# Jarvis73/PEMP

Measured on AMD Instinct MI355X. Metric: episodes/sec (PEMP stage-1 eval step, PASCAL-5i-shaped 1-shot, ResNet-50), higher is better.
Workload: dtype f32

## Files before the change

### pemp_amd/csrc/conv_common.h

```cpp
#pragma once
#include "common.h"

namespace pemp {

typedef __attribute__((ext_vector_type(16))) float f32x16;
typedef __attribute__((ext_vector_type(4))) float v4f;
typedef __attribute__((ext_vector_type(8))) __bf16 bf16x8;
typedef __attribute__((ext_vector_type(2))) unsigned int u32x2;

#define PEMP_CONV_BF16_IO 0x100u

__device__ __forceinline__ v4f load_quad(const float* base, size_t off, unsigned bf16) {
    if (!bf16) return *(const v4f*)(base + off);
    const u32x2 r = *(const u32x2*)((const unsigned short*)base + off);
    return v4f{__builtin_bit_cast(float, r.x << 16), __builtin_bit_cast(float, r.x & 0xFFFF0000u),
               __builtin_bit_cast(float, r.y << 16), __builtin_bit_cast(float, r.y & 0xFFFF0000u)};
}

__device__ __forceinline__ unsigned int bf16_bits(float f) {
    const unsigned int u = __builtin_bit_cast(unsigned int, f);
    if ((u & 0x7FFFFFFFu) > 0x7F800000u) return (u >> 16) | 0x40u;
    return (u + 0x7FFFu + ((u >> 16) & 1u)) >> 16;
}

// ... 224 lines not shown
                o.y = fmaxf(o.y, 0.f);
                o.z = fmaxf(o.z, 0.f);
                o.w = fmaxf(o.w, 0.f);
            }
            store_quad(a.y, (size_t)m * a.ldy + n, o, a.flags & PEMP_CONV_BF16_IO);
        }
    }
}

int launch_conv_dma(int tile, const ConvArgs& a, hipStream_t st);
bool conv_dma2_supported(const ConvArgs& a);
int launch_conv_dma2(int tile, const ConvArgs& a, hipStream_t st);
int launch_conv_dma2_group(int tile, ConvGroupArgs& g, hipStream_t st);
int launch_conv_dma2_hybrid(const ConvArgs& a, hipStream_t st);
int conv_dma2_hybrid_rows(int M, int Cout);
int launch_conv_dma2_bf16(int tile, const ConvArgs& a, hipStream_t st);
int launch_conv_dma2_db(int tile, ConvArgs a, void* ws, size_t ws_bytes, bool split, hipStream_t st);
int conv_dma2_tile_rows(int tile);
struct SplitKPlan { int full, split, pieces; size_t ws_bytes; };
SplitKPlan conv_dma2_splitk_plan(int tile, const ConvArgs& a);
int launch_conv_dma2_splitk(int tile, ConvArgs a, void* ws, size_t ws_bytes, hipStream_t st);
int launch_conv_dma2_split3(int tile, ConvArgs a, void* ws, size_t ws_bytes, bool split, hipStream_t st);
int launch_conv_dma2_group_split3(int tile, ConvGroupArgs& g, hipStream_t st);
int pack_split3(const float* w, void* out, int cout, int kpad, hipStream_t st);

}
```

### pemp_amd/csrc/conv_dma2.hip

```cpp
#include "conv_common.h"

#ifndef PEMP_SK_ACQUIRE
#define PEMP_SK_ACQUIRE 1
#endif

namespace pemp {

typedef __attribute__((address_space(3))) void* lptr_t;

template <int BM, int BN, int WGM, int NW, bool PADV, int EPI = 0, bool SK = false, bool BF16 = false, bool DB = false, bool R16 = false,
          bool S3 = false>
__device__ __forceinline__ void conv_dma2_body(const ConvArgs& a, const int bid, const int nblk) {
#if defined(__HIP_DEVICE_COMPILE__)
    constexpr int WGN = NW / WGM;
    constexpr int RPI = NW * 8;
    constexpr int WM = BM / WGM, WN = BN / WGN;
    static_assert(!R16 || (WM == 16 && WN % 16 == 0 && EPI == 0 && !SK && !BF16 && !DB), "R16: 16-row wave tiles, plain epilogue only");
    static_assert(!S3 || (EPI == 0 && !BF16 && !DB && !R16), "S3: plain epilogue, fp32 operands");
    constexpr int TM = R16 ? 1 : WM / 32, TN = R16 ? WN / 16 : WN / 32;
    constexpr int BQ = S3 ? 12 : 8;
    static_assert(!S3 || (BN * BQ) % (NW * 64) == 0, "S3: whole B DMA rounds");
    constexpr int AL = BM / RPI, BL = S3 ? BN * BQ / (NW * 64) : BN / RPI;
    constexpr int NMF = S3 ? 6 * TM * TN : R16 ? 2 * TN : TM * TN * (BF16 ? 1 : 4), NDS = S3 ? 2 * TM + 3 * TN : R16 ? 1 + TN : TM + TN,
                  NDMA = AL + BL;
// ... 211 lines not shown
                acc[mi][ni] = __builtin_amdgcn_mfma_f32_32x32x16_bf16(am_[mi], bm_, acc[mi][ni], 0, 0, 0);        \
                acc[mi][ni] = __builtin_amdgcn_mfma_f32_32x32x16_bf16(am_[mi], bh_, acc[mi][ni], 0, 0, 0);        \
                acc[mi][ni] = __builtin_amdgcn_mfma_f32_32x32x16_bf16(ah_[mi], bm_, acc[mi][ni], 0, 0, 0);        \
                acc[mi][ni] = __builtin_amdgcn_mfma_f32_32x32x16_bf16(ah_[mi], bh_, acc[mi][ni], 0, 0, 0);        \
            }                                                                                                     \
        } else if constexpr (R16) {        \
            _Pragma("unroll") for (int h_ = 0; h_ < 2; ++h_) _Pragma("unroll") for (int ni = 0; ni < TN; ++ni)    \
                acc16[ni] = __builtin_amdgcn_mfma_f32_16x16x4f32(a16[src_][h_], b16[src_][ni][h_], acc16[ni], 0, 0, 0); \
        } else                                                                                                    \
        _Pragma("unroll") for (int mi = 0; mi < TM; ++mi) _Pragma("unroll") for (int ni = 0; ni < TN; ++ni) {     \
            const v4f av = af[src_][mi], bv = bf[src_][ni];                                                       \
            if constexpr (BF16) {                                                                                 \
                acc[mi][ni] = __builtin_amdgcn_mfma_f32_32x32x16_bf16(__builtin_bit_cast(bf16x8, av),              \
                                                                      __builtin_bit_cast(bf16x8, bv), acc[mi][ni], 0, 0, 0); \
                continue;                                                                                         \
            }                                                                                                     \
            acc[mi][ni] = __builtin_amdgcn_mfma_f32_32x32x2f32(av.x, bv.x, acc[mi][ni], 0, 0, 0);                 \
            acc[mi][ni] = __builtin_amdgcn_mfma_f32_32x32x2f32(av.y, bv.y, acc[mi][ni], 0, 0, 0);                 \
            acc[mi][ni] = __builtin_amdgcn_mfma_f32_32x32x2f32(av.z, bv.z, acc[mi][ni], 0, 0, 0);                 \
            acc[mi][ni] = __builtin_amdgcn_mfma_f32_32x32x2f32(av.w, bv.w, acc[mi][ni], 0, 0, 0);                 \
        }                                                                                                         \
    } while (0)

#define PEMP_STEP(buf_, DMA_, NEXT_)                                                                              \
    do {                                                                                                          \
        PEMP_READ(1, buf_, 1);                                                                                    \
        __builtin_amdgcn_sched_barrier(0);                                                                        \
        PEMP_MMA(0);                                                                                              \
        __builtin_amdgcn_sched_barrier(0);                                                                        \
        if constexpr (!S3) {                                         \
            PEMP_READ(0, buf_, 2);                                                                                \
            __builtin_amdgcn_sched_barrier(0);                                                                    \
            PEMP_MMA(1);                                                                                          \
            __builtin_amdgcn_sched_barrier(0);                                                                    \
            PEMP_READ(1, buf_, 3);                                                                                \
            __builtin_amdgcn_sched_barrier(0);                                                                    \
            PEMP_MMA(0);                                                                                          \
            __builtin_amdgcn_sched_barrier(0);                                                                    \
        }                                                                                                         \
          \
        __builtin_amdgcn_s_waitcnt(0x0070);           \
        asm volatile("s_waitcnt vmcnt(0)" ::: "memory");       \
        __builtin_amdgcn_s_barrier();    \
        __builtin_amdgcn_sched_barrier(0);                                                                        \
        if (NEXT_) PEMP_READ(0, (buf_) ^ 1, 0);                                                                   \
        if (DMA_) {                                                                                               \
            PEMP_ADVANCE2();                                                                                      \
            PEMP_DMA2(buf_);                                                                                      \
        }                                                                                                         \
        PEMP_MMA(1);                          \
        if (DMA_) {                         \
            _Pragma("unroll") for (int k_ = 0; k_ < NMF; ++k_) {                                                  \
                __builtin_amdgcn_sched_group_barrier(0x008, 1, 0);                                                \
                _Pragma("unroll") for (int q_ = 0; q_ < PER; ++q_) {                                              \
                    const int it_ = k_ * PER + q_;                                                                \
                    if (it_ < NDS) __builtin_amdgcn_sched_group_barrier(0x100, 1, 0);                             \
                    else if (it_ < NDS + NDMA) __builtin_amdgcn_sched_group_barrier(0x020, 1, 0);                 \
                }                                                                                                 \
            }                                                                                                     \
        }                                                                                                         \
        __builtin_amdgcn_sched_barrier(0);                                                                        \
    } while (0)

    int kt = 0;
    PEMP_READ(0, 0, 0);
    for (; kt + 2 < nkl; ++kt) {
        const int buf = kt & 1;
        PEMP_STEP(buf, true, true);
    }
    if (kt + 1 < nkl) {
// ... 3 lines not shown
    }
    constexpr bool PRE = !R16 && TM * TN <= 2;
    v4f rpre[PRE ? TM * TN * 4 : 1];
#pragma unroll
    for (int i = 0; i < (PRE ? TM * TN * 4 : 1); ++i) rpre[i] = v4f{0.f, 0.f, 0.f, 0.f};
    if constexpr (PRE) {
        if (a.res) {
            const int rr_ = lane >> 3, c4_ = (lane & 7) * 4;
#pragma unroll
            for (int mi = 0; mi < TM; ++mi)
#pragma unroll
                for (int ni = 0; ni < TN; ++ni)
#pragma unroll
                    for (int i = 0; i < 4; ++i) {
                        const int m = m0 + wm0 + mi * 32 + rr_ + 8 * i, n = n0 + wn0 + ni * 32 + c4_;
                        rpre[(mi * TN + ni) * 4 + i] = m < a.M ? load_quad(a.res, (size_t)m * a.ldr + n, a.flags & PEMP_CONV_BF16_IO) : v4f{0.f, 0.f, 0.f, 0.f};
                    }
        }
    }
    {
        const int buf = kt & 1;
        PEMP_STEP(buf, false, false);
    }
#undef PEMP_STEP
#undef PEMP_DMA2
#undef PEMP_ADVANCE2
#undef PEMP_READ
#undef PEMP_MMA

    if constexpr (SK) {
        if (sk_r >= 0) {
            v4f* part = (v4f*)a.sk_ws + ((size_t)(sk_r * a.sk_S + piece) * NW + wave) * (TM * TN * 4 * 64) + lane;
#pragma unroll
            for (int mi = 0; mi < TM; ++mi)
#pragma unroll
                for (int ni = 0; ni < TN; ++ni)
#pragma unroll
                    for (int q = 0; q < 4; ++q) {
                        const v4f v = {acc[mi][ni][4 * q], acc[mi][ni][4 * q + 1], acc[mi][ni][4 * q + 2], acc[mi][ni][4 * q + 3]};
                        asm volatile("global_store_dwordx4 %0, %1, off sc0 sc1" ::"v"(part + ((mi * TN + ni) * 4 + q) * 64), "v"(v) : "memory");
                    }
            asm volatile("s_waitcnt vmcnt(0)" ::: "memory");
            __syncthreads();
            int* flag = (int*)smem;
            if (tid == 0) {
                const int v = __hip_atomic_fetch_add(a.sk_cnt + sk_r, 1, __ATOMIC_RELAXED, __HIP_MEMORY_SCOPE_AGENT);
#if PEMP_SK_ACQUIRE
                if (v == a.sk_S - 1) {
                    __builtin_amdgcn_fence(__ATOMIC_ACQUIRE, "agent");
                    asm volatile("s_waitcnt vmcnt(0)" ::: "memory");
                }
// ... 60 lines not shown

    float* Rall = (float*)smem + NW * 1024;
    static_assert(EPI == 0 || NW * 1024 + NW * TN * 512 <= 64 * (BM + BN), "LDS: statistics area");
    static_assert(NW * 1024 <= 64 * (BM + BN), "LDS: one 4 KB transpose patch per wave");
    if constexpr (R16) conv_epilogue_r16<TN>(a, acc16, (float*)smem + wave * 1024, m0 + wm0, n0 + wn0, lane);
    else if constexpr (PRE) conv_epilogue_lds_pre<TM, TN, TM * TN * 4, EPI, DB>(a, acc, (float*)smem + wave * 1024, m0 + wm0, n0 + wn0, lane, rpre, Rall + wave * TN * 512);
    else if constexpr (EPI != 0) {
        const v4f none[1] = {{0.f, 0.f, 0.f, 0.f}};
        conv_epilogue_lds_pre<TM, TN, 1, EPI>(a, acc, (float*)smem + wave * 1024, m0 + wm0, n0 + wn0, lane, none, Rall + wave * TN * 512);
    } else conv_epilogue_lds<TM, TN, DB>(a, acc, (float*)smem + wave * 1024, m0 + wm0, n0 + wn0, lane);
    if constexpr (EPI != 0) {
        __syncthreads();
        conv_stats_store<BN, WGM, NW, TN>(a, Rall, bm, n0, tid);
    }
#endif
}

template <int BM, int BN, int WGM, int NW, bool PADV, int EPI = 0, bool SK = false, bool BF16 = false, bool DB = false, bool R16 = false,
          bool S3 = false>
__global__ __launch_bounds__(NW * 64) void conv_dma2_kernel(ConvArgs a) {
    conv_dma2_body<BM, BN, WGM, NW, PADV, EPI, SK, BF16, DB, R16, S3>(a, blockIdx.x, gridDim.x);
}

template <int BM, int BN, int WGM, int NW, bool PADV, bool R16 = false, bool S3 = false>
__global__ __launch_bounds__(NW * 64) void conv_dma2_group_kernel(ConvGroupArgs g) {
    int which = 0;
#pragma unroll
    for (int i = 1; i < CONV_GROUP_MAX; ++i) which += (i < g.n && (int)blockIdx.x >= g.first[i]) ? 1 : 0;
    const int bid = (int)blockIdx.x - g.first[which];
    if (bid >= g.nblk[which]) return;
    conv_dma2_body<BM, BN, WGM, NW, PADV, 0, false, false, false, R16, S3>(g.a[which], bid, g.nblk[which]);
}

template <int BM, int BN, int WGM, int NW, bool R16 = false, bool S3 = false>
static int launch_dma2_group(ConvGroupArgs& g, bool padv, hipStream_t st) {
    const size_t lds = (size_t)2 * (8 * BM + (S3 ? 12 : 8) * BN) * sizeof(v4f);
    auto kern = padv ? conv_dma2_group_kernel<BM, BN, WGM, NW, true, R16, S3> : conv_dma2_group_kernel<BM, BN, WGM, NW, false, R16, S3>;
    if (lds > 64 * 1024) {
        hipError_t e = hipFuncSetAttribute((const void*)kern, hipFuncAttributeMaxDynamicSharedMemorySize, (int)lds);
        if (e != hipSuccess) {
            set_error("hipFuncSetAttribute(lds=%zu): %s", lds, hipGetErrorString(e));
            return (int)e;
        }
    }
    int grid = 0;
    for (int i = 0; i < g.n; ++i) {
        g.first[i] = grid;
        g.nblk[i] = cdiv(g.a[i].M, BM) * (g.a[i].Cout / BN);
        grid += (g.nblk[i] + 7) & ~7;
    }
    g.first[g.n] = grid;
    hipLaunchKernelGGL(kern, dim3(grid), dim3(NW * 64), lds, st, g);
    return launch_status("conv_dma2/group");
}

static int g_simds_of[64] = {0};

template <bool PADV>
__global__ __launch_bounds__(256) void conv_dma2_hybrid_kernel(ConvGroupArgs g) {
    const int bid = (int)blockIdx.x;
    if (bid < g.first[1]) {
        if (bid < g.nblk[0]) conv_dma2_body<64, 64, 2, 4, PADV, 0, false, false, false, false>(g.a[0], bid, g.nblk[0]);
    } else {
        conv_dma2_body<32, 64, 2, 4, PADV, 0, false, false, false, true>(g.a[1], bid - g.first[1], g.nblk[1]);
    }
}

int conv_dma2_hybrid_rows(int M, int Cout) {
    int dev = 0;
    if (hipGetDevice(&dev) != hipSuccess || dev < 0 || dev >= 64) dev = 63;
    if (!g_simds_of[dev]) {
        int cus = 0;
        if (dev == 63 || hipDeviceGetAttribute(&cus, hipDeviceAttributeMultiprocessorCount, dev) != hipSuccess || cus <= 0) cus = 256;
        g_simds_of[dev] = 4 * cus;
    }
    const int g_simds = g_simds_of[dev];
    if (M <= 0 || Cout < 64 || Cout % 64) return 0;
    const int per32 = Cout / 32;
    const int rounds = (int)(((long long)M / 32 * per32) / g_simds);
    if (rounds < 1 || rounds > 8) return 0;
    const int rows_a = ((long long)rounds * g_simds / per32) * 32 / 64 * 64;
    const int rest = M - rows_a;
    if (rows_a <= 0 || rest <= 0 || (long long)cdiv(rest, 16) * per32 > g_simds) return 0;
    return rows_a;
}

int launch_conv_dma2_hybrid(const ConvArgs& a, hipStream_t st) {
    if (a.stats || (a.flags & PEMP_CONV_BF16_IO)) return -2;
    const int rows_a = conv_dma2_hybrid_rows(a.M, a.Cout);
    if (!rows_a) return -2;
    const int rest = a.M - rows_a;
    ConvGroupArgs g;
    g.n = 2;
    g.a[0] = a;
    g.a[0].M = rows_a;
    g.a[1] = a;
    g.a[1].bm_first = rows_a / 32;
    for (int i = 2; i < CONV_GROUP_MAX; ++i) g.a[i] = a;
    g.nblk[0] = (rows_a / 64) * (a.Cout / 64);
// ... 206 lines not shown
    if (tile < 1 || tile > 6 || tile == 5 || a.stats || a.rowmask || (a.flags & PEMP_CONV_BF16_IO)) {
        set_error("conv split3: tile %d / epilogue outside the family", tile);
        return -1;
    }
    int bm, bn;
    tile_shape(tile, bm, bn);
    if (split) {
        const SplitKPlan p = conv_dma2_splitk_plan(tile, a);
        if (p.pieces >= 2) {
            if (!ws || ws_bytes < p.ws_bytes || ((uintptr_t)ws & 15)) {
                set_error("conv split-K: workspace of %zu bytes needed (16-byte aligned), got %zu", p.ws_bytes, ws_bytes);
                return -1;
            }
            a.sk_cnt = (int*)ws;
            a.sk_ws = (float*)((char*)ws + 1024);
            a.sk_full = p.full;
            a.sk_S = p.pieces;
            return launch_s3_tile<true>(tile, a, p.full + p.split * p.pieces, st);
        }
    }
    return launch_s3_tile<false>(tile, a, cdiv(a.M, bm) * (a.Cout / bn), st);
}

int launch_conv_dma2_group_split3(int tile, ConvGroupArgs& g, hipStream_t st) {
    if (tile == 5) {
        set_error("conv split3: no 128 x 64 8-wave form");
        return -1;
    }
    const bool padv = g.a[0].padv != nullptr;
    if (tile == 6) return launch_dma2_group<256, 128, 8, 8, false, true>(g, padv, st);
    if (tile == 4) return launch_dma2_group<128, 128, 4, 8, false, true>(g, padv, st);
    if (tile == 1) return launch_dma2_group<128, 128, 4, 4, false, true>(g, padv, st);
    if (tile == 2) return launch_dma2_group<128, 64, 4, 4, false, true>(g, padv, st);
    return launch_dma2_group<64, 64, 2, 4, false, true>(g, padv, st);
}

__global__ __launch_bounds__(256) void pack_split3_kernel(const float* __restrict__ w, unsigned short* __restrict__ out, long long n8) {
    const long long i = (long long)blockIdx.x * 256 + threadIdx.x;
    if (i >= n8) return;
    const v4f x0 = *(const v4f*)(w + i * 8), x1 = *(const v4f*)(w + i * 8 + 4);
    bf16x8 h, m, l;
    split3_bf16(x0, x1, h, m, l);
    const long long step = i >> 2;
    unsigned short* o = out + step * 96 + (i & 3) * 8;
    *(bf16x8*)o = h;
    *(bf16x8*)(o + 32) = m;
// ... 49 lines not shown
```

### pemp_amd/csrc/conv_igemm.hip

```cpp
#include "conv_common.h"

namespace pemp {


template <int BM, int BN, int WGM, bool STEM>
__global__ __launch_bounds__(256) void conv_igemm_kernel(ConvArgs a) {
    constexpr int WGN = 4 / WGM;
    constexpr int WM = BM / WGM, WN = BN / WGN;
    constexpr int TM = WM / 32, TN = WN / 32;
    constexpr int AL = BM / 32, BL = BN / 32;
    static_assert(TM >= 1 && TN >= 1, "wave tile");

    extern __shared__ __attribute__((aligned(16))) v4f smem[];
    v4f* As = smem;
    v4f* Bs = smem + 2 * 8 * BM;

    const int tid = threadIdx.x;
    const int lane = tid & 63;
    const int wave = tid >> 6;
    const int wm0 = (wave / WGN) * WM;
    const int wn0 = (wave % WGN) * WN;
    const int lr = lane & 31, lh = lane >> 5;

    const int ntn = a.Cout / BN;
// ... 258 lines not shown
    a.dil = d->dil; a.ldr = d->ldr; a.Kpad = d->Kpad; a.flags = d->flags;
    a.HoWo = d->Ho * d->Wo;
    a.M = d->N * a.HoWo;
    a.ntaps = ntaps;
    a.cin_steps = stem ? 1 : d->Cin / 32;
    a.nk = d->Kpad / 32;
    if (residual) PEMP_REQUIRE(d->ldr >= d->Cout && d->ldr % 4 == 0 && ((uintptr_t)residual & 15) == 0, "conv2d: ldr must be >= Cout and x4, residual 16-byte aligned");
    a.sk_ws = nullptr; a.sk_cnt = nullptr; a.sk_full = 0; a.sk_S = 1;
    a.bm_first = 0;
    return 0;
}

static int conv2d_impl(const pemp_conv_desc* d, const float* x, const float* w, float* y, const float* scale, const float* shift,
                       const float* residual, const float* pad_value, void* ws, size_t ws_bytes, void* stream) {
    ConvArgs a;
    const int rc = conv_fill(d, x, w, y, scale, shift, residual, pad_value, a);
    if (rc) return rc;
    const bool stem = d->flags & PEMP_CONV_STEM4;
    int tile = d->tile;
    if (tile == 0) {
        tile = 3;
    }
    hipStream_t st = (hipStream_t)stream;
    if ((tile >= 41 && tile <= 46) || (tile >= 51 && tile <= 56)) {
        PEMP_REQUIRE(tile != 53, "conv2d: no split-K variant of the 64 x 64 tile");
        PEMP_REQUIRE(tile != 45 && tile != 55, "conv2d: no split3 form of the 128 x 64 8-wave tile");
        PEMP_REQUIRE(!stem && conv_dma2_supported(a) && (long long)a.Cout * a.Kpad * 6 < (1ll << 31),
                     "conv2d: split3 tile %d needs a geometry of the buffer-addressed kernels (no stem, <= 32 taps, operands < 2 GiB)", tile);
        const int t = tile > 50 ? tile - 50 : tile - 40;
        PEMP_REQUIRE((t != 1 && t != 4 && t != 6) || a.Cout % 128 == 0, "conv2d: tile N=128 needs Cout %% 128 == 0");
        return launch_conv_dma2_split3(t, a, ws, ws_bytes, tile > 50, st);
    }
    if (tile >= 31 && tile <= 37) {
        PEMP_REQUIRE(tile != 33, "conv2d: no split-K variant of the 64 x 64 tile");
        if (conv_dma2_supported(a)) {
            const int t = tile - 30;
            PEMP_REQUIRE((t != 1 && t != 4 && t != 6) || a.Cout % 128 == 0, "conv2d: tile N=128 needs Cout %% 128 == 0");
            PEMP_REQUIRE(t != 7 || a.Cout % 256 == 0, "conv2d: tile 256x256 needs Cout %% 256 == 0");
            return launch_conv_dma2_splitk(t, a, ws, ws_bytes, st);
        }
        tile -= 20;
    }
    if (tile == 29) {
        if (conv_dma2_supported(a)) {
            const int rc2 = launch_conv_dma2_hybrid(a, st);
            if (rc2 != -2) return rc2;
        }
        tile = 23;
    }
    if (tile >= 21 && tile <= 28) {
        if (conv_dma2_supported(a)) {
// ... 208 lines not shown
```

### pemp_amd/ops.py

```python
import ctypes as C
import json
import os

import torch

from . import _lib
from ._lib import ConvDesc, CONV_RELU, CONV_SHIFT_PER_IMAGE, CONV_STEM4


def _stream():
    return C.c_void_p(torch.cuda.current_stream().cuda_stream)


def _p(t):
    return C.c_void_p(t.data_ptr()) if t is not None else C.c_void_p(0)


def _chk_dev(*ts):
    for t in ts:
        if t is not None and (not t.is_cuda):
            raise _lib.PempHipError("pemp_amd ops need device (cuda/HIP) tensors; there is no CPU path")


def _nhwc(t, name, dtype=torch.float32):
# ... 11 lines not shown
    if (w > 1 and h > 1 and t.stride(1) != w * ld) or (h * w > 1 and n > 1 and t.stride(0) != h * w * ld):
        raise ValueError(f"{name}: pixels must be densely packed with stride ld={ld}, got strides {t.stride()}")
    return ld


def conv_out_size(i, k, s, p, d):
    return (i + 2 * p - d * (k - 1) - 1) // s + 1


class ConvParams:
    __slots__ = ("w", "scale", "shift", "cin", "cout", "kh", "kw", "stride", "pad", "dil", "kpad", "stem", "relu", "w3")

    def __init__(self, w, scale, shift, cin, cout, kh, kw, stride, pad, dil, kpad, stem, relu, w3=None):
        self.w, self.scale, self.shift, self.w3 = w, scale, shift, w3
        self.cin, self.cout, self.kh, self.kw = cin, cout, kh, kw
        self.stride, self.pad, self.dil, self.kpad, self.stem, self.relu = stride, pad, dil, kpad, stem, relu


TILE_VARIANTS = {13: (64, 64), 14: (128, 128), 12: (128, 64), 11: (128, 128), 15: (128, 64), 3: (64, 64),
                 17: (256, 256), 16: (256, 128),
                 23: (64, 64), 24: (128, 128), 22: (128, 64), 21: (128, 128), 25: (128, 64), 27: (256, 256), 26: (256, 128),
                 28: (32, 64),
                 29: (64, 64)}
SPLIT3_TILES = (43, 42, 41, 44, 46)
SPLIT3_SPLITK_TILES = (51, 52, 54, 56)
SPLIT3_DEFAULT_TILE = 43
AUTOTUNE = True
PICK_HOOK = None
SPLITK = os.environ.get("PEMP_CONV_SPLITK", "1") != "0"
DEFAULT_TILE = 13
_TILE_CACHE = {}
_TILE_CACHE_FILE = os.environ.get("PEMP_TILE_CACHE")
WGRAD_PICKS = {}
if _TILE_CACHE_FILE and os.path.exists(_TILE_CACHE_FILE):
    with open(_TILE_CACHE_FILE) as _f:
        for _k, _v in json.load(_f).items():
            _key = json.loads(_k)
            if _key and _key[0] == "wgrad":
                WGRAD_PICKS[tuple(_key[1:])] = tuple(_v) if isinstance(_v, list) else int(_v)
            else:
                _TILE_CACHE[tuple(_key)] = int(_v)


def save_picks():
    if not _TILE_CACHE_FILE:
        return
    out = {json.dumps([int(v) for v in k]): t for k, t in _TILE_CACHE.items()}
# ... 66 lines not shown

    def timed(t, reps):
        launch(t)
        e0, e1 = torch.cuda.Event(enable_timing=True), torch.cuda.Event(enable_timing=True)
        e0.record()
        for _ in range(reps):
            launch(t)
        e1.record()
        e1.synchronize()
        return e0.elapsed_time(e1) / reps

    ms = {t: timed(t, 3) for t in cands}
    for t in cands:
        ms[t] = min(ms[t], timed(t, 3))
    top = sorted(cands, key=lambda t: ms[t])[:3]
    final = {t: min(timed(t, 8), timed(t, 8)) for t in top}
    best = min(top, key=lambda t: final[t])
    _TILE_CACHE[key] = best
    save_picks()
    return best


def _tile_bn(t):
    return TILE_VARIANTS[t - 30 if t > 50 else t - 20 if t > 40 else t - 10 if t > 30 else t][1]


def pack_split3(w):
    co, kpad = w.shape
    if w.dtype != torch.float32 or not w.is_contiguous() or kpad % 32:
        raise ValueError("pack_split3: a contiguous fp32 [Cout, Kpad] with Kpad % 32 == 0")
    out = torch.empty((co, kpad // 32, 3, 32), dtype=torch.bfloat16, device=w.device)
    _lib.check(_lib.load().pemp_pack_split3_bf16(_p(w), _p(out), co, kpad, _stream()), "pemp_pack_split3_bf16")
    return out


def hybrid_rows(n, ho, wo, cout):
    d = ConvDesc(n, ho, wo, 32, 32, ho, wo, cout, cout, 1, 1, 1, 0, 1, 0, 32, 0, 29)
    return int(_lib.load().pemp_conv2d_hybrid_rows(C.byref(d)))


def pack_conv_weight(w_oihw, stem4=False):
    co, ci, kh, kw = w_oihw.shape
    w = w_oihw.detach().permute(0, 2, 3, 1).contiguous().float()
    if stem4:
        if ci > 4:
            raise ValueError("stem4 packing needs Cin <= 4")
# ... 209 lines not shown
        keys += [p.cin, p.cout, p.kh, p.stride, p.pad, p.dil, nb, h, w, int(res is not None), int(pv is not None)]
    s3 = all(p.w3 is not None for p in ps)
    if not all(_group_member_ok(x, p, pv) for x, p, pv in zip(xs, ps, pad_values)) or (not s3 and any(p.w3 is not None for p in ps)):
        for x, p, out, pv, res in zip(xs, ps, outs, pad_values, residuals):
            conv2d(x, p, out=out, residual=res, pad_value=pv if p.kh * p.kw > 1 else None)
        return outs
    arr = lambda ts: (C.c_void_p * n)(*[(t.data_ptr() if t is not None else None) for t in ts])
    xa, wa, ya = arr(xs), arr([p.w3 if s3 else p.w for p in ps]), arr(outs)
    sa, ha, ra, pa = arr([p.scale for p in ps]), arr([p.shift for p in ps]), arr(residuals), arr(pad_values)
    ptr = lambda a: C.cast(a, C.POINTER(C.c_void_p))

    def launch(t):
        da = (ConvDesc * n)(*[ConvDesc(*d, t) for d in descs])
        _lib.check(lib.pemp_conv2d_group_nhwc_f32(n, da, ptr(xa), ptr(wa), ptr(ya), ptr(sa), ptr(ha), ptr(ra), ptr(pa), _stream()),
                   "pemp_conv2d_group_nhwc_f32")

    if tile == 0:
        key = (-8 if s3 else -7,) + tuple(keys)
        tile = _TILE_CACHE.get(key)
        if tile is None and s3:
            tile = SPLIT3_DEFAULT_TILE
            if _tunes(max(d[0] * d[5] * d[6] for d in descs)):
                tile = _pick_tile(launch, None, key, min(p.cout for p in ps),
                                  only=[t for t in SPLIT3_TILES if all(p.cout % _tile_bn(t) == 0 for p in ps)])
        if tile is None:
            if _tunes(max(d[0] * d[5] * d[6] for d in descs)):
                tile = _pick_tile(launch, None, key, min(p.cout for p in ps),
                                  only=[t for t in GROUP_TILES + (28,) if all(p.cout % TILE_VARIANTS[t][1] == 0 for p in ps)])
            else:
                tile = DEFAULT_TILE + 10
    launch(tile)
    return outs


SPLITK_TILES = (31, 32, 34, 35, 36, 37)
EVAL_SPLITK = os.environ.get("PEMP_EVAL_SPLITK", "0") == "1"
EVAL_SPLITK_MAX_ROWS = int(os.environ.get("PEMP_EVAL_SPLITK_MAX_ROWS", "12000"))
_SK_WS = {}
SK_SCOPE = 0
_SK_WS_BYTES = 72 << 20


class eval_splitk:

    def __init__(self, on=True):
        self.on = bool(on)

# ... 487 lines not shown
```

### scratch/s3_isa_mix.py

```python
import os
import re
import subprocess
import sys
import tempfile

ROOT = os.path.dirname(os.path.dirname(os.path.abspath(__file__)))
sys.path.insert(0, ROOT)

TILES = {43: (64, 64, 4), 42: (128, 64, 4), 41: (128, 128, 4), 44: (128, 128, 8), 46: (256, 128, 8)}
NAME = re.compile(r"^(_ZN4pemp16conv_dma2_kernelILi(\d+)ELi(\d+)ELi(\d+)ELi(\d+)ELb([01])ELi0ELb([01])ELb0ELb0ELb0ELb1EEEvNS_8ConvArgsE):")
NOT_SALU = ("s_waitcnt", "s_barrier", "s_nop", "s_cbranch", "s_branch", "s_setprio", "s_endpgm", "s_sleep")


def compile_asm(src):
    from pemp_amd import build
    out = tempfile.mkdtemp()
    asm = os.path.join(out, "conv_dma2.s")
    hipcc = os.environ.get("HIPCC", "/opt/rocm/bin/hipcc")
    r = subprocess.run([hipcc] + build.FLAGS + ["--cuda-device-only", "-S", src, "-o", asm, "-Rpass-analysis=kernel-resource-usage"],
                       capture_output=True, text=True, check=True)
    return asm, r.stderr


def resources(remarks):
    res, cur = {}, None
    for line in remarks.splitlines():
        m = re.search(r"remark: +Function Name: (\S+)", line)
        if m:
            cur = res.setdefault(m.group(1), {})
            continue
        m = re.search(r"remark: +([^:]+?): (\d+) \[", line)
        if m and cur is not None:
            cur[m.group(1)] = int(m.group(2))
    return res


def kernels(asm):
    out, cur, blocks = {}, None, None
    with open(asm) as f:
        for line in f:
            m = NAME.match(line)
            if m:
                cur = m.group(1)
                blocks = out[cur] = [("entry", [])]
                continue
            if cur is None:
                continue
            if line.startswith(".Lfunc_end"):
                cur = None
                continue
            s = line.strip()
            if re.match(r"^\.LBB\d+_\d+:", s):
                blocks.append((s[:-1].split(":")[0], []))
            elif s and not s.startswith((";", ".")):
                blocks[-1][1].append(s.split(";")[0].strip())
    return out


def mix(insts):
    ops = [i.split()[0] for i in insts if i]
    c = dict(mfma=sum(o.startswith("v_mfma") for o in ops),
             valu=sum(o.startswith("v_") and not o.startswith("v_mfma") for o in ops),
             cvt=sum(o == "v_cvt_pk_bf16_f32" for o in ops),
             salu=sum(o.startswith("s_") and not o.startswith(NOT_SALU) for o in ops),
# ... 7 lines not shown
    for label, insts in blocks:
        if not any(re.search(r"s_cbranch_\w+ " + re.escape(label) + r"$", i) for i in insts):
            continue
        c = mix(insts)
        if best is None or c["mfma"] > best["mfma"]:
            best = c
    return best


def main():
    args = [a for a in sys.argv[1:] if not a.startswith("--")]
    padv, sk = "--padv" in sys.argv, "--sk" in sys.argv
    src = args[0] if args else os.path.join(ROOT, "pemp_amd", "csrc", "conv_dma2.hip")
    remarks = ""
    if src.endswith(".hip"):
        asm, remarks = compile_asm(src)
    else:
        asm = src
    ks, res = kernels(asm), resources(remarks)
    print(f"{'id':>3} {'block / waves':>14} {'wave tile':>9} {'MFMA':>5} {'VALU':>5} {'cvt':>4} {'SALU':>5} {'ds_read':>7} {'VALU/MFMA':>9}"
          f" {'VGPR+AGPR':>9} {'scratch':>7} {'occ':>4}")
    for tid, (bm, bn, nw) in TILES.items():
        for name, blocks in ks.items():
            m = NAME.match(name + ":")
            if (int(m.group(2)), int(m.group(3)), int(m.group(5))) != (bm, bn, nw) or m.group(6) != str(int(padv)) or m.group(7) != str(int(sk)):
                continue
            wgm = int(m.group(4))
            wm, wn = bm // wgm, bn // (nw // wgm)
            c = kloop(blocks)
            steps = c["mfma"] // (6 * (wm // 32) * (wn // 32) * 2) if c else 0
            r = res.get(name, {})
            regs = (r.get("VGPRs", 0) + r.get("AGPRs", 0)) if r else "-"
            if not c or not steps:
                print(f"{tid:>3} no K loop found in {name}")
                continue
            per = {k: v / steps for k, v in c.items()}
            print(f"{tid:>3} {f'{bm}x{bn} / {nw}':>14} {f'{wm}x{wn}':>9} {per['mfma']:>5.0f} {per['valu']:>5.0f} {per['cvt']:>4.0f} {per['salu']:>5.0f}"
                  f" {per['ds_read']:>7.0f} {per['valu'] / per['mfma']:>9.2f} {regs:>9} {r.get('ScratchSize [bytes/lane]', '-'):>7}"
                  f" {r.get('Occupancy [waves/SIMD]', '-'):>4}")


if __name__ == "__main__":
    main()
```

### scratch/s3_layers_bench.py

```python
import argparse
import hashlib
import os
import sys

import torch

sys.path.insert(0, os.path.dirname(os.path.dirname(os.path.abspath(__file__))))
from pemp_amd import ops

UNSPLIT = (43, 42, 41, 44, 46)
SPLIT = (52, 51, 54, 56)
LAYERS = ((256, 1024, 1, 1, True, False), (512, 1024, 1, 1, False, False), (1024, 256, 1, 1, False, False),
          (256, 256, 3, 2, False, False), (128, 512, 1, 1, True, False), (1024, 512, 1, 1, False, False),
          (256, 256, 3, 2, False, True))


def timed(fn, reps, n=5):
    for _ in range(2):
        fn()
    e0, e1 = torch.cuda.Event(enable_timing=True), torch.cuda.Event(enable_timing=True)
    best = 1e9
    for _ in range(reps):
        e0.record()
        for _ in range(n):
            fn()
        e1.record()
        e1.synchronize()
        best = min(best, e0.elapsed_time(e1) / n * 1e3)
    return best


def digest(t):
    return hashlib.sha1(t.cpu().numpy().tobytes()).hexdigest()[:16]
# ... 51 lines not shown
```

Measured before the change: 1331.

## Add persistent split3 conv kernel overlapping next-tile DMA with epilogue

```diff
diff --git a/pemp_amd/csrc/conv_common.h b/pemp_amd/csrc/conv_common.h
--- a/pemp_amd/csrc/conv_common.h
+++ b/pemp_amd/csrc/conv_common.h
@@ -270,6 +270,8 @@
 int launch_conv_dma2_splitk(int tile, ConvArgs a, void* ws, size_t ws_bytes, hipStream_t st);
 int launch_conv_dma2_split3(int tile, ConvArgs a, void* ws, size_t ws_bytes, bool split, hipStream_t st);
 int launch_conv_dma2_group_split3(int tile, ConvGroupArgs& g, hipStream_t st);
+int launch_conv_dma2_split3_persist(int tile, const ConvArgs& a, hipStream_t st);
+int conv_dma2_simds();
 int pack_split3(const float* w, void* out, int cout, int kpad, hipStream_t st);
 
 }
diff --git a/pemp_amd/csrc/conv_dma2.hip b/pemp_amd/csrc/conv_dma2.hip
--- a/pemp_amd/csrc/conv_dma2.hip
+++ b/pemp_amd/csrc/conv_dma2.hip
@@ -257,7 +257,8 @@
         }                                                                                                         \
     } while (0)
 
-#define PEMP_STEP(buf_, DMA_, NEXT_)                                                                              \
+#define PEMP_STEP(buf_, DMA_, NEXT_) PEMP_STEP_X(buf_, DMA_, NEXT_, true, true)
+#define PEMP_STEP_X(buf_, DMA_, NEXT_, ADV_, WVM_)                                                                \
     do {                                                                                                          \
         PEMP_READ(1, buf_, 1);                                                                                    \
         __builtin_amdgcn_sched_barrier(0);                                                                        \
@@ -274,13 +275,18 @@
             __builtin_amdgcn_sched_barrier(0);                                                                    \
         }                                                                                                         \
           \
-        __builtin_amdgcn_s_waitcnt(0x0070);           \
-        asm volatile("s_waitcnt vmcnt(0)" ::: "memory");       \
+        if (WVM_) {                                                                                               \
+            __builtin_amdgcn_s_waitcnt(0x0070);       \
+            asm volatile("s_waitcnt vmcnt(0)" ::: "memory");    \
+        } else {                                                                                                  \
+            __builtin_amdgcn_s_waitcnt(0xC07F);                         \
+            asm volatile("s_waitcnt lgkmcnt(0)" ::: "memory");                                                    \
+        }                                                                                                         \
         __builtin_amdgcn_s_barrier();    \
         __builtin_amdgcn_sched_barrier(0);                                                                        \
         if (NEXT_) PEMP_READ(0, (buf_) ^ 1, 0);                                                                   \
         if (DMA_) {                                                                                               \
-            PEMP_ADVANCE2();                                                                                      \
+            if (ADV_) PEMP_ADVANCE2();                                                                            \
             PEMP_DMA2(buf_);                                                                                      \
         }                                                                                                         \
         PEMP_MMA(1);                          \
@@ -330,11 +336,6 @@
         const int buf = kt & 1;
         PEMP_STEP(buf, false, false);
     }
-#undef PEMP_STEP
-#undef PEMP_DMA2
-#undef PEMP_ADVANCE2
-#undef PEMP_READ
-#undef PEMP_MMA
 
     if constexpr (SK) {
         if (sk_r >= 0) {
@@ -441,6 +442,269 @@
     conv_dma2_body<BM, BN, WGM, NW, PADV, EPI, SK, BF16, DB, R16, S3>(a, blockIdx.x, gridDim.x);
 }
 
+template <int TM, int TN>
+__device__ __forceinline__ void conv_epilogue_s3p(const ConvArgs& a, f32x16 (&acc)[TM][TN], float* S, int m_base, int n_base,
+                                                  int lane, const v4f (&pre)[TM * TN * 4], const v4f (&scv)[TN], const v4f (&shv)[TN]) {
+    const bool relu = a.flags & PEMP_CONV_RELU;
+    const bool per_img = a.flags & PEMP_CONV_SHIFT_PER_IMAGE;
+    const int lr = lane & 31, lh = lane >> 5;
+    const int rr = lane >> 3, c4 = (lane & 7) * 4;
+#pragma unroll
+    for (int ni = 0; ni < TN; ++ni) {
+        const int n = n_base + ni * 32 + c4;
+        const v4f sc = scv[ni], sh = shv[ni];
+#pragma unroll
+        for (int mi = 0; mi < TM; ++mi) {
+#pragma unroll
+            for (int e = 0; e < 16; ++e) S[((e & 3) + 8 * (e >> 2) + 4 * lh) * 32 + lr] = acc[mi][ni][e];
+            asm volatile("s_waitcnt lgkmcnt(0)" ::: "memory");
+#pragma unroll
+            for (int i = 0; i < 4; ++i) {
+                const int row = rr + 8 * i;
+                const int m = m_base + mi * 32 + row;
+                const v4f v = *(const v4f*)(S + row * 32 + c4);
+                if (m < a.M) {
+                    v4f add = sh;
+                    if (per_img) add += *(const v4f*)(a.shift + (size_t)(m / a.HoWo) * a.Cout + n);
+                    if (a.res) add += pre[(mi * TN + ni) * 4 + i];
+                    v4f o;
+                    o.x = __builtin_fmaf(v.x, sc.x, add.x);
+                    o.y = __builtin_fmaf(v.y, sc.y, add.y);
+                    o.z = __builtin_fmaf(v.z, sc.z, add.z);
+                    o.w = __builtin_fmaf(v.w, sc.w, add.w);
+                    if (relu) {
+                        o.x = fmaxf(o.x, 0.f);
+                        o.y = fmaxf(o.y, 0.f);
+                        o.z = fmaxf(o.z, 0.f);
+                        o.w = fmaxf(o.w, 0.f);
+                    }
+                    store_quad(a.y, (size_t)m * a.ldy + n, o, a.flags & PEMP_CONV_BF16_IO);
+                }
+            }
+            asm volatile("s_waitcnt lgkmcnt(0)" ::: "memory");
+        }
+    }
+}
+
+template <int BM, int BN, int WGM, int NW, bool PADV>
+__device__ __forceinline__ void conv_dma2_s3p_body(const ConvArgs& a) {
+#if defined(__HIP_DEVICE_COMPILE__)
+    constexpr bool S3 = true, R16 = false, BF16 = false;
+    constexpr int WGN = NW / WGM;
+    constexpr int RPI = NW * 8;
+    constexpr int WM = BM / WGM, WN = BN / WGN;
+    constexpr int TM = WM / 32, TN = WN / 32;
+    constexpr int BQ = 12;
+    static_assert((BN * BQ) % (NW * 64) == 0, "S3: whole B DMA rounds");
+    constexpr int AL = BM / RPI, BL = BN * BQ / (NW * 64);
+    constexpr int NMF = 6 * TM * TN, NDS = 2 * TM + 3 * TN, NDMA = AL + BL;
+    constexpr int PER = (NDS + NDMA + NMF - 1) / NMF;
+    constexpr int NST = TM * TN * 4;
+    static_assert(NDMA + NST <= 63, "vmcnt range");
+    static_assert(NW <= BM / 32 + 3 * BN / 64, "one 4 KB transpose patch per wave inside ONE stage buffer");
+
+    extern __shared__ __attribute__((aligned(16))) v4f smem[];
+    v4f* As = smem;
+    v4f* Bs = smem + 2 * BM * 8;
+
+    const int tid = threadIdx.x;
+    const int lane = tid & 63;
+    const int wave = __builtin_amdgcn_readfirstlane(tid >> 6);
+    const int wm0 = (wave / WGN) * WM;
+    const int wn0 = (wave % WGN) * WN;
+    const int lr = lane & 31, lh = lane >> 5;
+
+    const int ntn = a.Cout / BN;
+    const int T = (a.M + BM - 1) / BM * ntn;
+    const int xcd = (int)blockIdx.x & 7, idx = (int)blockIdx.x >> 3;
+    const int q8 = T >> 3, r8 = T & 7;
+    const int t_first = xcd < r8 ? xcd * (q8 + 1) : r8 * (q8 + 1) + (xcd - r8) * q8;
+    const int t_cnt = q8 + (xcd < r8 ? 1 : 0);
+    const int gx = ((int)gridDim.x - xcd + 7) >> 3;
+    if (idx >= t_cnt) return;
+    int j = idx;
+    int m0 = (a.bm_first + (t_first + j) / ntn) * BM, n0 = ((t_first + j) % ntn) * BN;
+
+    const int p = tid & 7;
+    const int r = tid >> 3;
+    const int sq = p ^ ((r >> 1) & 7);
+    const int bias_pix = a.pad * a.W + a.pad;
+    const __amdgpu_buffer_rsrc_t rx =
+        __builtin_amdgcn_make_buffer_rsrc((void*)(a.x - (ptrdiff_t)bias_pix * a.ldx), 0, 0x80000000u, 0x00020000);
+    const __amdgpu_buffer_rsrc_t rw = __builtin_amdgcn_make_buffer_rsrc((void*)a.w, 0, 0x80000000u, 0x00020000);
+    const unsigned padv_off = PADV ? (unsigned)((const char*)a.padv - (const char*)(a.x - (ptrdiff_t)bias_pix * a.ldx)) + sq * 16 : 0x80000000u;
+    unsigned a_voff[AL], a_inv[AL], b_voff[BL];
+    auto offsets = [&](const int m0_, const int n0_) {
+#pragma unroll
+        for (int i = 0; i < AL; ++i) {
+            const int m = m0_ + r + RPI * i;
+            const bool ok = m < a.M;
+            const int mm = ok ? m : 0;
+            const int img = mm / a.HoWo;
+            const int rem = mm - img * a.HoWo;
+            const int ho = rem / a.Wo;
+            const int wo = rem - ho * a.Wo;
+            const int hi0 = ho * a.stride - a.pad;
+            const int wi0 = wo * a.stride - a.pad;
+            a_voff[i] = (unsigned)(((img * a.H + hi0) * a.W + wi0 + bias_pix) * a.ldx + sq * 4) * 4u;
+            unsigned mask = 0;
+            int kh = 0, kw = 0;
+            for (int t = 0; t < a.ntaps; ++t) {
+                const int hi = hi0 + kh * a.dil, wi = wi0 + kw * a.dil;
+                if (ok && (unsigned)hi < (unsigned)a.H && (unsigned)wi < (unsigned)a.W) mask |= 1u << t;
+                if (++kw == a.KW) {
+                    kw = 0;
+                    ++kh;
+                }
+            }
+            a_inv[i] = ~mask;
+        }
+#pragma unroll
+        for (int i = 0; i < BL; ++i) {
+            const int q = i * NW * 64 + tid, row = q / 12, pos = q - row * 12;
+            const int src = (pos & ~3) | ((pos & 3) ^ ((row >> 2) & 3));
+            b_voff[i] = (unsigned)((n0_ + row) * a.Kpad * 6 + src * 16);
+        }
+    };
+    offsets(m0, n0);
+
+    int tap = 0, cb = 0, kh_i = 0, kw_i = 0;
+    const int tapw = a.dil * a.ldx * 4, taph = a.dil * a.W * a.ldx * 4;
+    int multi, s_kw, s_ntaps;
+    asm volatile("s_nop 0\n\tv_readfirstlane_b32 %0, %3\n\tv_readfirstlane_b32 %1, %4\n\tv_readfirstlane_b32 %2, %5\n\ts_nop 4"
+                 : "=s"(multi), "=s"(s_kw), "=s"(s_ntaps)
+                 : "v"(a.ntaps > 1 ? 1 : 0), "v"(a.KW), "v"(a.ntaps));
+    const int nkl = a.nk;
+
+    PEMP_DMA2(0);
+    if (nkl > 1) {
+        PEMP_ADVANCE2();
+        PEMP_DMA2(1);
+        asm volatile("s_waitcnt vmcnt(%0)" ::"n"(NDMA) : "memory");
+    } else {
+        asm volatile("s_waitcnt vmcnt(0)" ::: "memory");
+    }
+    __builtin_amdgcn_s_barrier();
+    __builtin_amdgcn_sched_barrier(0);
+
+    const int rsw = (lr >> 1) & 7;
+    const int arow = (wm0 + lr) * 8, brow = (wn0 + lr) * 8;
+    v4f af[2][1], bf[2][1];
+    const int r16 = lane & 15, g16 = lane >> 4;
+    const int rsw16 = (r16 >> 1) & 7;
+    const int arow16 = (wm0 + r16) * 32 + (g16 >> 1), brow16 = (wn0 + r16) * 32 + (g16 >> 1);
+    float a16[2][2], b16[2][1][2];
+    v4f acc16[1];
+    v4f af3[2][TM][2], bf3[2][TN][3];
+    const int brow3 = (wn0 + lr) * 12, bsw3 = (lr >> 2) & 3;
+    const int rr_ = lane >> 3, c4_ = (lane & 7) * 4;
+
+    int pb = 0;
+    for (;;) {
+        f32x16 acc[TM][TN];
+#pragma unroll
+        for (int mi = 0; mi < TM; ++mi)
+#pragma unroll
+            for (int ni = 0; ni < TN; ++ni)
+#pragma unroll
+                for (int e = 0; e < 16; ++e) acc[mi][ni][e] = 0.f;
+        const int jn = j + gx;
+        const bool more = jn < t_cnt;
+        const int m0n = more ? (a.bm_first + (t_first + jn) / ntn) * BM : m0, n0n = more ? ((t_first + jn) % ntn) * BN : n0;
+
+        int kt = 0;
+        PEMP_READ(0, pb, 0);
+        for (; kt + 2 < nkl; ++kt) {
+            const int buf = (kt + pb) & 1;
+            PEMP_STEP(buf, true, true);
+        }
+        if (more) {
+            offsets(m0n, n0n);
+        } else {
+#pragma unroll
+            for (int i = 0; i < AL; ++i) {
+                a_voff[i] = 0x80000000u;
+                a_inv[i] = 0u;
+            }
+#pragma unroll
+            for (int i = 0; i < BL; ++i) b_voff[i] = 0x80000000u;
+        }
+        tap = 0;
+        cb = 0;
+        kh_i = 0;
+        kw_i = 0;
+        if (kt + 1 < nkl) {
+            const int buf = (kt + pb) & 1;
+            PEMP_STEP_X(buf, true, true, false, true);
+            ++kt;
+        }
+        const int bl = (kt + pb) & 1;
+        v4f rres[TM * TN * 4], scv[TN], shv[TN];
+        auto epi_loads = [&]() {
+            const bool per_img = a.flags & PEMP_CONV_SHIFT_PER_IMAGE;
+#pragma unroll
+            for (int ni = 0; ni < TN; ++ni) {
+                const int n = n0 + wn0 + ni * 32 + c4_;
+                scv[ni] = a.scale ? *(const v4f*)(a.scale + n) : v4f{1.f, 1.f, 1.f, 1.f};
+                shv[ni] = (a.shift && !per_img) ? *(const v4f*)(a.shift + n) : v4f{0.f, 0.f, 0.f, 0.f};
+            }
+#pragma unroll
+            for (int i = 0; i < TM * TN * 4; ++i) rres[i] = v4f{0.f, 0.f, 0.f, 0.f};
+            if (a.res) {
+#pragma unroll
+                for (int mi = 0; mi < TM; ++mi)
+#pragma unroll
+                    for (int ni = 0; ni < TN; ++ni)
+#pragma unroll
+                        for (int i = 0; i < 4; ++i) {
+                            const int m = m0 + wm0 + mi * 32 + rr_ + 8 * i, n = n0 + wn0 + ni * 32 + c4_;
+                            rres[(mi * TN + ni) * 4 + i] = m < a.M ? load_quad(a.res, (size_t)m * a.ldr + n, a.flags & PEMP_CONV_BF16_IO)
+                                                                   : v4f{0.f, 0.f, 0.f, 0.f};
+                        }
+            }
+        };
+        PEMP_STEP_X(bl, false, false, true, false);
+        epi_loads();
+
+        float* patch = wave < BM / 32 ? (float*)(As + bl * BM * 8 + wave * 256) : (float*)(Bs + bl * BN * BQ + (wave - BM / 32) * 256);
+        conv_epilogue_s3p<TM, TN>(a, acc, patch, m0 + wm0, n0 + wn0, lane, rres, scv, shv);
+        if (!more) {
+            asm volatile("s_waitcnt vmcnt(0)" ::: "memory");
+            break;
+        }
+
+        const int pbn = (pb + nkl) & 1;
+        __builtin_amdgcn_s_barrier();
+        if (nkl > 1) {
+            PEMP_ADVANCE2();
+            PEMP_DMA2(bl);
+            if (m0 + wm0 + WM <= a.M) asm volatile("s_waitcnt vmcnt(%0)" ::"n"(NDMA + NST) : "memory");
+            else asm volatile("s_waitcnt vmcnt(%0)" ::"n"(NDMA) : "memory");
+        } else {
+            PEMP_DMA2(pbn);
+            asm volatile("s_waitcnt vmcnt(0)" ::: "memory");
+        }
+        __builtin_amdgcn_s_barrier();
+        __builtin_amdgcn_sched_barrier(0);
+        j = jn;
+        m0 = m0n;
+        n0 = n0n;
+        pb = pbn;
+    }
+#endif
+}
+
+template <int BM, int BN, int WGM, int NW, bool PADV>
+__global__ __launch_bounds__(NW * 64) __attribute__((amdgpu_waves_per_eu(BM == 64 ? 4 : 2))) void conv_dma2_s3p_kernel(ConvArgs a) {
+    conv_dma2_s3p_body<BM, BN, WGM, NW, PADV>(a);
+}
+#undef PEMP_STEP_X
+#undef PEMP_STEP
+#undef PEMP_DMA2
+#undef PEMP_ADVANCE2
+#undef PEMP_READ
+#undef PEMP_MMA
+
 template <int BM, int BN, int WGM, int NW, bool PADV, bool R16 = false, bool S3 = false>
 __global__ __launch_bounds__(NW * 64) void conv_dma2_group_kernel(ConvGroupArgs g) {
     int which = 0;
@@ -485,7 +749,7 @@
     }
 }
 
-int conv_dma2_hybrid_rows(int M, int Cout) {
+int conv_dma2_simds() {
     int dev = 0;
     if (hipGetDevice(&dev) != hipSuccess || dev < 0 || dev >= 64) dev = 63;
     if (!g_simds_of[dev]) {
@@ -493,7 +757,11 @@
         if (dev == 63 || hipDeviceGetAttribute(&cus, hipDeviceAttributeMultiprocessorCount, dev) != hipSuccess || cus <= 0) cus = 256;
         g_simds_of[dev] = 4 * cus;
     }
-    const int g_simds = g_simds_of[dev];
+    return g_simds_of[dev];
+}
+
+int conv_dma2_hybrid_rows(int M, int Cout) {
+    const int g_simds = conv_dma2_simds();
     if (M <= 0 || Cout < 64 || Cout % 64) return 0;
     const int per32 = Cout / 32;
     const int rounds = (int)(((long long)M / 32 * per32) / g_simds);
@@ -746,6 +1014,45 @@
     return launch_s3_tile<false>(tile, a, cdiv(a.M, bm) * (a.Cout / bn), st);
 }
 
+template <int BM, int BN, int WGM, int NW>
+static int launch_dma2_s3p(const ConvArgs& a, hipStream_t st) {
+    const size_t lds = (size_t)2 * (8 * BM + 12 * BN) * sizeof(v4f);
+    auto kern = a.padv ? conv_dma2_s3p_kernel<BM, BN, WGM, NW, true> : conv_dma2_s3p_kernel<BM, BN, WGM, NW, false>;
+    if (lds > 64 * 1024) {
+        hipError_t e = hipFuncSetAttribute((const void*)kern, hipFuncAttributeMaxDynamicSharedMemorySize, (int)lds);
+        if (e != hipSuccess) {
+            set_error("hipFuncSetAttribute(lds=%zu): %s", lds, hipGetErrorString(e));
+            return (int)e;
+        }
+    }
+    static int occ[2] = {0, 0};
+    int& o = occ[a.padv ? 1 : 0];
+    if (!o) {
+        int v = 0;
+        hipError_t e = hipOccupancyMaxActiveBlocksPerMultiprocessor(&v, (const void*)kern, NW * 64, lds);
+        if (e != hipSuccess || v <= 0) {
+            set_error("conv split3 persistent: occupancy query failed (%s, %d blocks)", hipGetErrorString(e), v);
+            return -1;
+        }
+        o = v;
+    }
+    const long long tiles = (long long)cdiv(a.M, BM) * (a.Cout / BN);
+    long long grid = (long long)o * (conv_dma2_simds() / 4);
+    if (grid < 8) grid = 8;
+    if (grid > tiles) grid = tiles;
+    hipLaunchKernelGGL(kern, dim3((unsigned)grid), dim3(NW * 64), lds, st, a);
+    return launch_status("conv_dma2/split3/persistent");
+}
+
+int launch_conv_dma2_split3_persist(int tile, const ConvArgs& a, hipStream_t st) {
+    if (a.stats || a.rowmask || (a.flags & PEMP_CONV_BF16_IO)) {
+        set_error("conv split3: tile %d / epilogue outside the family", tile);
+        return -1;
+    }
+    if (tile == 9) return launch_dma2_s3p<256, 128, 8, 8>(a, st);
+    return launch_dma2_s3p<64, 64, 2, 4>(a, st);
+}
+
 int launch_conv_dma2_group_split3(int tile, ConvGroupArgs& g, hipStream_t st) {
     if (tile == 5) {
         set_error("conv split3: no 128 x 64 8-wave form");
diff --git a/pemp_amd/csrc/conv_igemm.hip b/pemp_amd/csrc/conv_igemm.hip
--- a/pemp_amd/csrc/conv_igemm.hip
+++ b/pemp_amd/csrc/conv_igemm.hip
@@ -304,11 +304,16 @@
         tile = 3;
     }
     hipStream_t st = (hipStream_t)stream;
-    if ((tile >= 41 && tile <= 46) || (tile >= 51 && tile <= 56)) {
+    if ((tile >= 41 && tile <= 49) || (tile >= 51 && tile <= 56)) {
         PEMP_REQUIRE(tile != 53, "conv2d: no split-K variant of the 64 x 64 tile");
         PEMP_REQUIRE(tile != 45 && tile != 55, "conv2d: no split3 form of the 128 x 64 8-wave tile");
+        PEMP_REQUIRE(tile != 48, "conv2d: no persistent split3 form of the 128 x 128 4-wave tile");
         PEMP_REQUIRE(!stem && conv_dma2_supported(a) && (long long)a.Cout * a.Kpad * 6 < (1ll << 31),
                      "conv2d: split3 tile %d needs a geometry of the buffer-addressed kernels (no stem, <= 32 taps, operands < 2 GiB)", tile);
+        if (tile == 47 || tile == 49) {
+            PEMP_REQUIRE(tile == 47 || a.Cout % 128 == 0, "conv2d: tile N=128 needs Cout %% 128 == 0");
+            return launch_conv_dma2_split3_persist(tile - 40, a, st);
+        }
         const int t = tile > 50 ? tile - 50 : tile - 40;
         PEMP_REQUIRE((t != 1 && t != 4 && t != 6) || a.Cout % 128 == 0, "conv2d: tile N=128 needs Cout %% 128 == 0");
         return launch_conv_dma2_split3(t, a, ws, ws_bytes, tile > 50, st);
diff --git a/pemp_amd/ops.py b/pemp_amd/ops.py
--- a/pemp_amd/ops.py
+++ b/pemp_amd/ops.py
@@ -57,7 +57,8 @@
                  23: (64, 64), 24: (128, 128), 22: (128, 64), 21: (128, 128), 25: (128, 64), 27: (256, 256), 26: (256, 128),
                  28: (32, 64),
                  29: (64, 64)}
-SPLIT3_TILES = (43, 42, 41, 44, 46)
+SPLIT3_TILES = (43, 42, 41, 44, 46, 47, 49)
+SPLIT3_PERSISTENT = {47: 43, 49: 46}
 SPLIT3_SPLITK_TILES = (51, 52, 54, 56)
 SPLIT3_DEFAULT_TILE = 43
 AUTOTUNE = True
@@ -170,6 +171,7 @@
 
 
 def _tile_bn(t):
+    t = SPLIT3_PERSISTENT.get(t, t)
     return TILE_VARIANTS[t - 30 if t > 50 else t - 20 if t > 40 else t - 10 if t > 30 else t][1]
 
 
@@ -425,7 +427,7 @@
             tile = SPLIT3_DEFAULT_TILE
             if _tunes(max(d[0] * d[5] * d[6] for d in descs)):
                 tile = _pick_tile(launch, None, key, min(p.cout for p in ps),
-                                  only=[t for t in SPLIT3_TILES if all(p.cout % _tile_bn(t) == 0 for p in ps)])
+                                  only=[t for t in SPLIT3_TILES if t not in SPLIT3_PERSISTENT and all(p.cout % _tile_bn(t) == 0 for p in ps)])
         if tile is None:
             if _tunes(max(d[0] * d[5] * d[6] for d in descs)):
                 tile = _pick_tile(launch, None, key, min(p.cout for p in ps),
diff --git a/scratch/s3_isa_mix.py b/scratch/s3_isa_mix.py
--- a/scratch/s3_isa_mix.py
+++ b/scratch/s3_isa_mix.py
@@ -7,8 +7,10 @@
 ROOT = os.path.dirname(os.path.dirname(os.path.abspath(__file__)))
 sys.path.insert(0, ROOT)
 
-TILES = {43: (64, 64, 4), 42: (128, 64, 4), 41: (128, 128, 4), 44: (128, 128, 8), 46: (256, 128, 8)}
+TILES = {43: (64, 64, 4), 42: (128, 64, 4), 41: (128, 128, 4), 44: (128, 128, 8), 46: (256, 128, 8), 47: (64, 64, 4), 49: (256, 128, 8)}
+PERSISTENT = (47, 49)
 NAME = re.compile(r"^(_ZN4pemp16conv_dma2_kernelILi(\d+)ELi(\d+)ELi(\d+)ELi(\d+)ELb([01])ELi0ELb([01])ELb0ELb0ELb0ELb1EEEvNS_8ConvArgsE):")
+NAME_P = re.compile(r"^(_ZN4pemp20conv_dma2_s3p_kernelILi(\d+)ELi(\d+)ELi(\d+)ELi(\d+)ELb([01])()EEEvNS_8ConvArgsE):")
 NOT_SALU = ("s_waitcnt", "s_barrier", "s_nop", "s_cbranch", "s_branch", "s_setprio", "s_endpgm", "s_sleep")
 
 
@@ -39,7 +41,7 @@
     out, cur, blocks = {}, None, None
     with open(asm) as f:
         for line in f:
-            m = NAME.match(line)
+            m = NAME.match(line) or NAME_P.match(line)
             if m:
                 cur = m.group(1)
                 blocks = out[cur] = [("entry", [])]
@@ -93,8 +95,12 @@
           f" {'VGPR+AGPR':>9} {'scratch':>7} {'occ':>4}")
     for tid, (bm, bn, nw) in TILES.items():
         for name, blocks in ks.items():
-            m = NAME.match(name + ":")
-            if (int(m.group(2)), int(m.group(3)), int(m.group(5))) != (bm, bn, nw) or m.group(6) != str(int(padv)) or m.group(7) != str(int(sk)):
+            m = (NAME_P if tid in PERSISTENT else NAME).match(name + ":")
+            if not m or (int(m.group(2)), int(m.group(3)), int(m.group(5))) != (bm, bn, nw) or m.group(6) != str(int(padv)):
+                continue
+            if tid in PERSISTENT and sk:
+                continue
+            if tid not in PERSISTENT and m.group(7) != str(int(sk)):
                 continue
             wgm = int(m.group(4))
             wm, wn = bm // wgm, bn // (nw // wgm)
diff --git a/scratch/s3_layers_bench.py b/scratch/s3_layers_bench.py
--- a/scratch/s3_layers_bench.py
+++ b/scratch/s3_layers_bench.py
@@ -8,7 +8,7 @@
 sys.path.insert(0, os.path.dirname(os.path.dirname(os.path.abspath(__file__))))
 from pemp_amd import ops
 
-UNSPLIT = (43, 42, 41, 44, 46)
+UNSPLIT = (43, 42, 41, 44, 46, 47, 49)
 SPLIT = (52, 51, 54, 56)
 LAYERS = ((256, 1024, 1, 1, True, False), (512, 1024, 1, 1, False, False), (1024, 256, 1, 1, False, False),
           (256, 256, 3, 2, False, False), (128, 512, 1, 1, True, False), (1024, 512, 1, 1, False, False),
```

New measurement: 1387, median of 6. 1.04x the previous value.
